# cvg/diffmvs

Hardware: AMD Instinct MI355X
Metric: depth-maps/sec (640x512, 5 src views) (higher is better)
Workload: dtype f32

## Files before the change

diffmvs_amd/_lib.py:

```python
from __future__ import annotations

import ctypes as C
import os

PKG = os.path.dirname(os.path.abspath(__file__))
HIP_LIB_PATH = os.environ.get("DMVS_LIB") or os.path.join(PKG, "libdmvs_hip.so")

ACT_NONE, ACT_RELU, ACT_SIGMOID, ACT_TANH, ACT_SILU = range(5)
IN_PLAIN, IN_UPSAMPLE2, IN_UNSHUFFLE2, IN_ZEROINSERT2 = range(4)
LAYOUT_NCHW, LAYOUT_NHWC, LAYOUT_NHWC_BF16, LAYOUT_NHWC_F16 = 0, 1, 2, 3
DTYPE_F32, DTYPE_BF16, DTYPE_F16, DTYPE_F32_PLAIN = 0, 1, 2, 3
ARITH_F32, ARITH_BF16, ARITH_SPLIT = 0, 1, 2
EW_DEPTH_TO_DISP, EW_DISP_TO_DEPTH = 0, 1

_P = C.c_void_p
_I = C.c_int32
_F = C.c_float


class Conv2dDesc(C.Structure):
    _fields_ = [
        ("in0", _P), ("in1", _P), ("mul0", _P), ("weight", _P), ("scale", _P), ("shift", _P),
        ("residual", _P), ("gru_z", _P), ("gru_h", _P), ("out", _P), ("gn_stats", _P), ("out_mul", _P),
        ("B", _I), ("c0", _I), ("c1", _I), ("Hin", _I), ("Win", _I), ("Hout", _I), ("Wout", _I),
        ("cout", _I), ("cout_pad", _I), ("kh", _I), ("kw", _I), ("stride", _I), ("pad_h", _I), ("pad_w", _I),
        ("in_mode", _I), ("act", _I), ("res_mode", _I), ("res_after_act", _I),
        ("out_layout", _I), ("out_cstride", _I), ("out_coffset", _I), ("gn_groups", _I), ("post_scale", _F),
        ("gate_cstride", _I), ("arith", _I), ("tune", _I), ("out_mul_c0", _I), ("in0_cstride", _I), ("weight_split", _P),
    ]


class Conv3dDesc(C.Structure):
    _fields_ = [
        ("in_", _P), ("weight", _P), ("scale", _P), ("shift", _P), ("residual", _P), ("out", _P),
        ("B", _I), ("cin", _I), ("cout", _I), ("cout_pad", _I),
        ("Din", _I), ("Hin", _I), ("Win", _I), ("Dout", _I), ("Hout", _I), ("Wout", _I),
        ("stride", _I), ("transposed", _I), ("act", _I), ("tune", _I),
    ]


class GetCostDesc(C.Structure):
    _fields_ = [
        ("ref", _P), ("src", _P), ("rt", _P), ("inv_depth", _P), ("confidence", _P), ("view_w", _P),
        ("disp_min", _P), ("disp_max", _P), ("out_cost", _P), ("out_samples", _P), ("worklist", _P),
        ("B", _I), ("S", _I), ("C", _I), ("G", _I), ("n", _I), ("H", _I), ("W", _I), ("vw_shift", _I),
        ("cost_cstride", _I), ("cost_coffset", _I), ("samp_cstride", _I), ("samp_coffset", _I),
        ("interval", _F), ("min_radius", _F), ("max_radius", _F), ("feat_dtype", _I), ("tune", _I),
    ]


SIGNATURES = {
    "dmvs_abi_version": [],
    "dmvs_conv2d_f32": [C.POINTER(Conv2dDesc), _P],
    "dmvs_featurenet_stem_f32": [_P, _P, _P, _P, _P, _P, _P, _P, _I, _I, _I, _I, _P],
    "dmvs_featurenet_stem3_f32": [_P, _P, _P, _P, _P, _P, _P, _P, _P, _P, _P, _I, _I, _I, _I, _P],
    "dmvs_conv2d_wgrad_workspace_f32": [C.POINTER(Conv2dDesc), C.POINTER(C.c_int64)],
    "dmvs_conv2d_wgrad_f32": [C.POINTER(Conv2dDesc), _P, _P, _P, _P, C.c_int64, _P],
    "dmvs_conv3d_f32": [C.POINTER(Conv3dDesc), _P],
    "dmvs_conv3d_wgrad_workspace_f32": [C.POINTER(Conv3dDesc), C.POINTER(C.c_int64)],
    "dmvs_conv3d_wgrad_f32": [C.POINTER(Conv3dDesc), _P, _P, _P, _P, C.c_int64, _P],
    "dmvs_compose_proj_f32": [_P, _P, _I, _I, _P],
    "dmvs_warp_volume_f32": [_P, _P, _P, _P, _I, _I, _I, _I, _I, _I, _I, _P],
    "dmvs_getcost_quad_f32": [C.POINTER(GetCostDesc), _P],
    "dmvs_warp_corr_init_quad_f32": [_P, _P, _P, _P, _P, _P, _I, _I, _I, _I, _I, _I, _I, _I, _I, _I, _I, _P],
    "dmvs_warp_corr_init_bwd_f32": [_P, _P, _P, _P, _P, _P, _P, _P, _I, _I, _I, _I, _I, _I, _I, _I, _I, _I, _P],
    "dmvs_getcost_bwd_f32": [C.POINTER(GetCostDesc), _P, _P, _P, _P],
    "dmvs_view_aggregate_bwd_f32": [_P, _P, _P, _P, _P, _P, _I, _I, _I, _I, _P],
    "dmvs_view_aggregate_f32": [_P, _P, _P, _I, _I, _I, _I, _P],
    "dmvs_sigmoid_max_d_f32": [_P, _P, _I, _I, _I, _P],
    "dmvs_depth_regress_f32": [_P, _P, _P, _P, _P, _P, _I, _I, _I, _P],
    "dmvs_convex_upsample_f32": [_P, _P, _P, _P, _P, _P, _I, _I, _I, _I, _P],
    "dmvs_mask_upsample4_f32": [_P, _P, _P, _F, _P, _P, _P, _P, _P, _I, _I, _I, _I, _I, _P],
    "dmvs_groupnorm_silu_f32": [_P, _P, _P, _P, _P, _P, _P, _I, _I, _I, _I, _F, _P],
    "dmvs_groupnorm_apply_f32": [_P, _P, _P, _P, _P, _P, _P, _I, _I, _I, _I, _F, _P],
    "dmvs_delta_update_f32": [_P, _P, _P, _F, _P, _P, _P, _I, _I, _I, _I, _P],
    "dmvs_depth_convert_f32": [_P, _P, _P, _P, _I, _I, _I, _P],
    "dmvs_act_slice_f32": [_P, _P, _I, _I, _I, _I, _I, _I, _I, _I, _P],
    "dmvs_upsample_nearest_f32": [_P, _P, _I, _I, _I, _I, _P],
    "dmvs_nchw_to_nhwc_f32": [_P, _P, _I, _I, _I, _P],
    "dmvs_groupnorm_silu_bwd_workspace_f32": [_I, _I, _I, C.POINTER(C.c_int64)],
    "dmvs_groupnorm_silu_bwd_f32": [_P, _P, _P, _P, _P, _P, _P, _P, _P, _P, _P, C.c_int64, _I, _I, _I, _I, _F, _P],
    "dmvs_batchnorm_workspace_f32": [_I, _I, _I, _I, C.POINTER(C.c_int64)],
    "dmvs_batchnorm_train_fwd_f32": [_P, _P, _P, _P, _P, _P, _P, _P, _P, C.c_int64, _I, _I, _I, _I, _I, _F, _F, _I, _P],
    "dmvs_batchnorm_train_bwd_f32": [_P, _P, _P, _P, _P, _P, _P, _P, _P, _P, C.c_int64, _I, _I, _I, _I, _I, _I, _P],
    "dmvs_geo_consistency_f32": [_P, _P, _P, _P, _P, _I, _I, _F, _F, _P, _P, _I, _I, _I, _I, _I, _P],
    "dmvs_sumsq_f32": [_P, C.c_int64, _P, _P],
    "dmvs_adamw_step_f32": [_P, _P, _P, _P, C.c_int64, _F, _F, _F, _F, _F, _I, _F, _P, _F, _P],
    "dmvs_view_select_scores_f64": [_P, _P, _P, _P, _P, C.c_int64, C.c_int64, _P, _I, C.c_double, C.c_double, C.c_double, _P, _P, _P],
    "dmvs_cloud_nn_dist_f32": [_P, C.c_int64, _P, C.c_int64, _P, _P, C.c_int64, _P, C.c_double, _P, _F, _P, _P, _P],
    "dmvs_cloud_stats_f32": [_P, _P, C.c_int64, _F, _P, _I, C.c_double, _I, _P, _P],
    "dmvs_cloud_nn_index_f32": [_P, C.c_int64, _P, C.c_int64, _P, _P, C.c_int64, _P, C.c_double, _P, _F, _P, _P, _P, _P, _P],
    "dmvs_cloud_pair_moments_f64": [_P, C.c_int64, _P, _P, C.c_int64, _P, _P, _F, _P, _P, C.c_double, C.c_double, C.c_double, _I, _P, _P],
    "dmvs_cloud_crop_prism_f32": [_P, C.c_int64, _P, _P, _I, _I, C.c_double, C.c_double, _P, _P],
    "dmvs_depth_stats_f32": [_P, _P, _P, C.c_int64, C.c_int64, _P, _I, C.c_double, C.c_double, C.c_double, C.c_double, _I, _P, _P],
    "dmvs_cloud_splat_zmin_f32": [_P, C.c_int64, _P, _P, C.c_int64, _I, _I, C.c_double, C.c_double, C.c_double, _I, _I, _P, _P, _P, _P],
    "dmvs_cloud_splat_sum_f32": [_P, C.c_int64, _P, _P, C.c_int64, _I, _I, C.c_double, C.c_double, C.c_double, C.c_double, C.c_double, _I, _P, _P, _P, _P],
    "dmvs_depth_normals_f32": [_P, _P, _P, C.c_int64, _I, _I, _I, C.c_double, _I, _P, _P, _P],
}
VIEW_SELECT_MAX_IMAGES, VIEW_SELECT_MAX_LIST = 16384, 1 << 23
CLOUD_MAX_RINGS, CLOUD_MAX_KEY_BITS, CLOUD_MAX_THRESHOLDS = 1024, 62, 16
CLOUD_MOMENTS, CLOUD_MAX_POLYGON = 20, 256
DEPTH_MAX_THRESHOLDS, DEPTH_SLOTS = 8, 7
SPLAT_VIEW_CHUNK, SPLAT_VIEW_DOUBLES, SPLAT_SLOTS, SPLAT_MAX_RADIUS, SPLAT_NO_PRETEST = 8, 15, 4, 16, 0x1
NORMAL_MAX_RADIUS, NORMAL_CAM_DOUBLES, NORMAL_VIEW_CHUNK, NORMAL_SLOTS = 4, 27, 8, 4
ABI_VERSION = 4
TUNE_NO_WALK, TUNE_PIECES4, TUNE_NO_LEAN, TUNE_1X1_TILED, TUNE_NO_TALL, TUNE_TALL = 0x4, 0x8, 0x100, 0x200, 0x400, 0x800
TUNE3D_PIECES4, TUNE3D_S2_DIRECT, TUNE3D_NO_PAIR = 0x1, 0x2, 0x4
TUNE_SWEEP_GLOBAL = 0x1
TUNE_WGRAD_ACCUMULATE = 0x1000
TUNE_SPLIT_ALL = 0x20000
TUNE_STEM_EXACT = 0x40000


def tune_xcd_group(n: int) -> int:
    return (int(n) & 7) << 14


def tune3d_xcd_group(n: int) -> int:
    return (int(n) & 7) << 4
TUNE_BWD_INTERLEAVED, BWD_GATHER_INTERLEAVED = 0x1, 2


def tune_tile_wx(n: int) -> int:
    return n & 3


def tune_tile_mt(n: int) -> int:
    return (n & 7) << 4


class DmvsError(RuntimeError):
    pass


class Lib:

    def __init__(self, path: str):
        if not os.path.exists(path):
# ... 27 lines not shown
```

diffmvs_amd/build.py:

```python
from __future__ import annotations

import os
import subprocess
import sys

PKG = os.path.dirname(os.path.abspath(__file__))
ROOT = os.path.dirname(PKG)
CSRC = os.path.join(PKG, "csrc")
LIB = os.path.join(PKG, "libdmvs_hip.so")
PROBE_LIB = os.path.join(PKG, "libdmvs_probe.so")
PROBE_SOURCES = ["probe/getcost_probe.hip", "probe/random_line_gather.hip"]
SOURCES = ["conv2d_k33.hip", "conv2d_k55.hip", "conv2d_k77.hip", "conv2d_k15.hip", "conv2d.hip", "stem.hip", "stem3.hip", "conv3d.hip", "warp_quad.hip", "warp_bwd.hip", "warp_bwd_win.hip", "warp_init_bwd_win.hip", "misc.hip", "mask_upsample.hip", "optim.hip", "norm.hip", "fusion.hip", "view_select.hip", "cloud_eval.hip", "cloud_register.hip", "depth_eval.hip", "cloud_render.hip", "depth_normals.hip"]


def _deps():
    out = [os.path.join(ROOT, "include", "dmvs.h"), os.path.join(ROOT, "include", "dmvs_probe.h")]
    for base, _, files in os.walk(CSRC):
        out += [os.path.join(base, f) for f in files]
    return out


def _stale() -> bool:
    if not os.path.exists(LIB) or not os.path.exists(PROBE_LIB):
        return True
    t = min(os.path.getmtime(LIB), os.path.getmtime(PROBE_LIB))
    return any(os.path.getmtime(d) > t for d in _deps())


def build_hip(force: bool = False, save_temps: bool = False, verbose: bool = True) -> str:
    if not force and not _stale():
        return LIB
    import time
    t_start = time.time()
    hipcc = os.environ.get("HIPCC", "/opt/rocm/bin/hipcc")
    flags = ["--offload-arch=gfx950", "-O3", "-std=c++17", "-fPIC",
             "-I", os.path.join(ROOT, "include"), "-I", CSRC,
             "-munsafe-fp-atomics",
             "-Wall", "-Wno-unused-function"]
    objdir = os.path.join(ROOT, "build", "temps" if save_temps else "obj")
    os.makedirs(objdir, exist_ok=True)
    if save_temps:
        flags += ["-save-temps=obj", "-Rpass-analysis=kernel-resource-usage"]

    hdr_t = max(os.path.getmtime(d) for d in _deps() if d.endswith(".h"))

    def compile_one(src):
        obj = os.path.join(objdir, src.replace("/", "_") + ".o")
        if not force and not save_temps and os.path.exists(obj) and os.path.getmtime(obj) > max(hdr_t, os.path.getmtime(os.path.join(CSRC, src))):
            return obj
        cmd = [hipcc] + flags + ["-c", os.path.join(CSRC, src), "-o", obj]
        if verbose:
            print("[diffmvs_amd.build]", " ".join(cmd), flush=True)
        t0 = time.time()
        subprocess.run(cmd, check=True, cwd=objdir if save_temps else ROOT)
        os.utime(obj, (t0, t0))
        return obj

    from concurrent.futures import ThreadPoolExecutor
    with ThreadPoolExecutor(max_workers=min(len(SOURCES), os.cpu_count() or 4)) as pool:
        objs = list(pool.map(compile_one, SOURCES + PROBE_SOURCES))
    for lib, lobjs in ((LIB, objs[:len(SOURCES)]), (PROBE_LIB, objs[len(SOURCES):])):
        link = [hipcc, "--offload-arch=gfx950", "-shared", "-fPIC"] + lobjs + ["-o", lib]
        if verbose:
            print("[diffmvs_amd.build]", " ".join(link), flush=True)
        subprocess.run(link, check=True, cwd=ROOT)
        os.utime(lib, (t_start, t_start))
    return LIB


if __name__ == "__main__":
    build_hip(force="--force" in sys.argv, save_temps="--save-temps" in sys.argv)
    print(LIB)
```

diffmvs_amd/engine.py:

```python
from __future__ import annotations

import math
import os
from typing import Callable, Dict, List, Optional

import torch
import torch.nn.functional as F

from . import ops as K
from .ops import Ops, PackedConv, pack_conv2d, pack_conv3d

_RATIOS = [4, 2, 1]
_MULTS = [(1,), (1, 2), (1, 2, 4)]


def _bn(sd, p):
    return {k: sd[f"{p}.{k}"] for k in ("weight", "bias", "running_mean", "running_var")}


def _cw(sd, p, **kw):
    return pack_conv2d(sd[p + ".conv.weight"], sd.get(p + ".conv.bias"),
                       bn=_bn(sd, p + ".bn") if (p + ".bn.weight") in sd else None, **kw)


def pack_feature(sd, p="feature", g4=False, feat_dtype=torch.float32):
    order = (lambda w: w[K.g4_channels(w.shape[0], feat_dtype).to(w.device)].contiguous()) if g4 else (lambda w: w)
    f = {"conv0.0": _cw(sd, p + ".conv0.0", pad=1), "conv0.1": _cw(sd, p + ".conv0.1", pad=1)}
    for i in (1, 2, 3):
        f[f"conv{i}.0"] = _cw(sd, f"{p}.conv{i}.0", stride=2, pad=2)
        f[f"conv{i}.1"], f[f"conv{i}.2"] = _cw(sd, f"{p}.conv{i}.1", pad=1), _cw(sd, f"{p}.conv{i}.2", pad=1)
    f["out1"] = pack_conv2d(order(sd[p + ".out1.weight"]))
    f["inner1"] = pack_conv2d(sd[p + ".inner1.weight"], sd[p + ".inner1.bias"])
    f["out2"] = pack_conv2d(order(sd[p + ".out2.weight"]), pad=1)
    if (p + ".out3.weight") in sd:
        f["inner2"] = pack_conv2d(sd[p + ".inner2.weight"], sd[p + ".inner2.bias"])
        f["out3"] = pack_conv2d(order(sd[p + ".out3.weight"]), pad=1)
    return f


STEM_FUSE_DEFAULT = "1"


def stem3_applies(o: Ops, x):
    return (o.conv_arith == K.ARITH_SPLIT and os.environ.get("DMVS_STEM_FUSE", STEM_FUSE_DEFAULT) != "0" and
            o.featurenet_stem3_supported(x))


def run_feature(o: Ops, f, x, layout=K.LAYOUT_NHWC, feat_dtype=torch.float32):
    R = K.ACT_RELU
    if stem3_applies(o, x):
        c1 = o.featurenet_stem3(f["conv0.0"], f["conv0.1"], f["conv1.0"], x)
    else:
        c0 = o.featurenet_stem(f["conv0.0"], f["conv0.1"], x)
        c1 = o.conv2d(f["conv1.0"], c0, act=R)
    c1 = o.conv2d(f["conv1.2"], o.conv2d(f["conv1.1"], c1, act=R), act=R)
    c2 = o.conv2d(f["conv2.2"], o.conv2d(f["conv2.1"], o.conv2d(f["conv2.0"], c1, act=R), act=R), act=R)
    c3 = o.conv2d(f["conv3.2"], o.conv2d(f["conv3.1"], o.conv2d(f["conv3.0"], c2, act=R), act=R), act=R)
    out = {"stage1": o.conv2d(f["out1"], c3, out_layout=layout, out_dtype=feat_dtype)}
    intra = o.conv2d(f["inner1"], c2, residual=c3, res_mode=K.IN_UPSAMPLE2)
    out["stage2"] = o.conv2d(f["out2"], intra, out_layout=layout, out_dtype=feat_dtype)
    if "out3" in f:
        intra = o.conv2d(f["inner2"], c1, residual=intra, res_mode=K.IN_UPSAMPLE2)
        out["stage3"] = o.conv2d(f["out3"], intra, out_layout=layout, out_dtype=feat_dtype)
    return out


def pack_context_trunk(sd, p="context"):
    c = {"conv1": _cw(sd, p + ".conv1", pad=1)}
    for li in (1, 2, 3):
        for bi in (0, 1):
            q = f"{p}.layer{li}.{bi}"
            c[f"{li}.{bi}.conv1"] = _cw(sd, q + ".conv1", stride=(2 if bi == 0 else 1), pad=1)
            c[f"{li}.{bi}.conv2"] = _cw(sd, q + ".conv2", pad=1)
            if bi == 0:
                c[f"{li}.{bi}.down"] = _cw(sd, q + ".downsample", stride=2, pad=1)
    return c


def run_context_trunk(o: Ops, c, x):
    R = K.ACT_RELU
    x = o.conv2d(c["conv1"], x, act=R)
    taps = {}
    for li in (1, 2, 3):
        y = o.conv2d(c[f"{li}.0.conv1"], x, act=R)
        xd = o.conv2d(c[f"{li}.0.down"], x)
        x = o.conv2d(c[f"{li}.0.conv2"], y, residual=xd, act=R)
        y = o.conv2d(c[f"{li}.1.conv1"], x, act=R)
        x = o.conv2d(c[f"{li}.1.conv2"], y, residual=x, act=R)
        taps[3 - li] = x
    return taps


def pack_pvw(sd, p):
    return (pack_conv3d(sd[p + ".conv.0.conv.weight"], bn=_bn(sd, p + ".conv.0.bn")),
            pack_conv3d(sd[p + ".conv.1.weight"], sd[p + ".conv.1.bias"]))


def run_pvw(o: Ops, pk, cor):
    N, _, D, H, W = cor.shape
    x = o.conv3d(pk[1], o.conv3d(pk[0], cor, act=K.ACT_RELU))
    return o.sigmoid_max_d(x.view(N, D, H, W))


def pack_costreg(sd, p):
    reg = {}
    for i, st in ((0, 1), (1, 1), (2, 2), (3, 1), (4, 2), (5, 1)):
        reg[i] = pack_conv3d(sd[f"{p}.conv{i}.conv.weight"], bn=_bn(sd, f"{p}.conv{i}.bn"), stride=st)
    for i in (6, 7):
        reg[i] = pack_conv3d(sd[f"{p}.conv{i}.conv.weight"], bn=_bn(sd, f"{p}.conv{i}.bn"), stride=2, transposed=True)
    reg["prob"] = pack_conv3d(sd[p + ".prob.weight"])
    return reg


def run_costreg(o: Ops, reg, x):
    R = K.ACT_RELU
    c1 = o.conv3d(reg[1], o.conv3d(reg[0], x, act=R), act=R)
    c3 = o.conv3d(reg[3], o.conv3d(reg[2], c1, act=R), act=R)
    x = o.conv3d(reg[5], o.conv3d(reg[4], c3, act=R), act=R)
    x = o.conv3d(reg[6], x, act=R, residual=c3)
    x = o.conv3d(reg[7], x, act=R, residual=c1)
    return o.conv3d(reg["prob"], x)


def pack_mask(sd, p):
    return (pack_conv2d(sd[p + ".0.weight"], sd[p + ".0.bias"], pad=1), pack_conv2d(sd[p + ".2.weight"], sd[p + ".2.bias"]))


def run_mask(o: Ops, pk, context, post_scale=0.25):
    return o.conv2d(pk[1], o.conv2d(pk[0], context, act=K.ACT_RELU), post_scale=post_scale)


def mask_head_fuses(pk, up_ratio) -> bool:
    return up_ratio == 4 and pk[1].cin == 64 and pk[1].cout == 144 and pk[1].scale is None and os.environ.get("DMVS_MASK_FUSE", "1") != "0"


def pack_gru(sd, p):
    g = {}
    for n, pad in (("1", (0, 2)), ("2", (2, 0))):
# ... 439 lines not shown
```

diffmvs_amd/ops.py:

```python
from __future__ import annotations

import ctypes as C
import os
from dataclasses import dataclass
from typing import Optional

import torch

from . import _lib
from ._lib import (ACT_NONE, ACT_RELU, ACT_SIGMOID, ACT_SILU, ACT_TANH, ARITH_BF16, ARITH_F32, ARITH_SPLIT, DTYPE_BF16, DTYPE_F16, DTYPE_F32, IN_PLAIN,
                   IN_UNSHUFFLE2, IN_UPSAMPLE2, IN_ZEROINSERT2, LAYOUT_NCHW, LAYOUT_NHWC, LAYOUT_NHWC_BF16, LAYOUT_NHWC_F16)

CONV_ARITH = {"fp32": ARITH_F32, "bf16": ARITH_BF16, "split": ARITH_SPLIT}
FEATURE_DTYPES = {"fp32": torch.float32, "bf16": torch.bfloat16, "fp16": torch.float16}
_DTYPE_CODE = {torch.float32: DTYPE_F32, torch.bfloat16: DTYPE_BF16, torch.float16: DTYPE_F16}
_NHWC_LAYOUT = {torch.float32: LAYOUT_NHWC, torch.bfloat16: LAYOUT_NHWC_BF16, torch.float16: LAYOUT_NHWC_F16}


def _round_up(x: int, m: int) -> int:
    return (x + m - 1) // m * m


@dataclass
class PackedConv:
# ... 246 lines not shown
            c0, Hin, Win = x0.shape[1], x0.shape[2] * 2, x0.shape[3] * 2
        else:
            c0, Hin, Win = x0.shape[1] * 4, x0.shape[2] // 2, x0.shape[3] // 2
        c1 = 0 if x1 is None else x1.shape[1]
        assert c0 + c1 == pc.cin, (c0, c1, pc.cin)
        kh, kw = pc.k
        Hout = (Hin + 2 * pc.pad[0] - kh) // pc.stride + 1
        Wout = (Win + 2 * pc.pad[1] - kw) // pc.stride + 1
        if out_cstride is None:
            out_cstride = pc.cout
        if out is None:
            shape = (B, out_cstride, Hout, Wout) if out_layout == LAYOUT_NCHW else (B, Hout, Wout, out_cstride)
            out = self.empty(*shape, dtype=out_dtype)
        arith = self.conv_arith if arith is None else arith
        wsplit = split_weights(pc) if (arith == ARITH_SPLIT and kh * kw > 1 and out_layout in (LAYOUT_NCHW, LAYOUT_NHWC)) else None
        d = _lib.Conv2dDesc(
            weight_split=_ptr(wsplit),
            in0=_ptr(x0), in1=_ptr(x1), mul0=_ptr(mul0), weight=_ptr(pc.weight), scale=_ptr(pc.scale),
            shift=_ptr(pc.shift), residual=_ptr(residual), gru_z=_ptr(gru_z), gru_h=_ptr(gru_h), out=_ptr(out),
            gn_stats=_ptr(gn_stats), gn_groups=(gn_groups if gn_stats is not None else 0), B=B, c0=c0, c1=c1, Hin=Hin, Win=Win, Hout=Hout, Wout=Wout, cout=pc.cout, cout_pad=pc.cout_pad,
            kh=kh, kw=kw, stride=pc.stride, pad_h=pc.pad[0], pad_w=pc.pad[1], in_mode=in_mode, act=act,
            res_mode=res_mode, res_after_act=int(res_after_act), out_layout=out_layout, out_cstride=out_cstride,
            out_coffset=out_coffset, post_scale=post_scale, gate_cstride=gate_cstride,
            arith=arith, tune=(self.tune["conv2d"] if tune is None else tune),
            out_mul=_ptr(out_mul), out_mul_c0=out_mul_c0, in0_cstride=in0_cstride)
        self._call("dmvs_conv2d_f32", C.byref(d), self.stream())
        if self.timers is not None and "dmvs_conv2d_f32" in self.timers:
            self.timers.setdefault("_conv2d_flops", []).append(2.0 * B * Hout * Wout * pc.cout * pc.cin * kh * kw)
            self.timers.setdefault("_conv2d_shape", []).append((B, pc.cin, pc.cout, kh, kw, pc.stride, Hout, Wout, in_mode, int(mul0 is not None)))
            nb = sum(t.numel() * t.element_size() for t in (x0, x1, mul0, residual, gru_z, gru_h, out_mul) if t is not None)
            self.timers.setdefault("_conv2d_bytes", []).append(nb + B * Hout * Wout * pc.cout * out.element_size())
        return out

    def featurenet_stem(self, pc0: PackedConv, pc1: PackedConv, x, tune=None):
        if isinstance(x, (list, tuple)):
            self._chk(*x)
            Bv, cin, H, W = x[0].shape
            y = self.empty(len(x) * Bv, 8, H, W)
            for v, xv in enumerate(x):
                self._stem_launch(pc0, pc1, xv, y[v * Bv:(v + 1) * Bv], tune)
            return y
        self._chk(x)
        N, cin, H, W = x.shape
        y = self.empty(N, 8, H, W)
        self._stem_launch(pc0, pc1, x, y, tune)
        return y

    def _stem_launch(self, pc0: PackedConv, pc1: PackedConv, x, y, tune=None):
        N, cin, H, W = x.shape
        if not (cin == 3 and pc0.cin == 3 and pc0.cout == 8 and pc1.cin == 8 and pc1.cout == 8 and pc0.k == (3, 3) and
                pc1.k == (3, 3) and pc0.stride == 1 and pc1.stride == 1 and pc0.pad == (1, 1) and pc1.pad == (1, 1) and
                pc0.cout_pad == 8 and pc1.cout_pad == 8):
            raise _lib.DmvsError("featurenet_stem: expects the 3->8->8 3x3 stem of FeatureNet")
        tune = self.tune["stem"] if tune is None else tune
        if self.conv_arith != ARITH_SPLIT:
            tune |= _lib.TUNE_STEM_EXACT
        self._call("dmvs_featurenet_stem_f32", _ptr(x), _ptr(pc0.weight), _ptr(pc0.scale), _ptr(pc0.shift), _ptr(pc1.weight),
                   _ptr(pc1.scale), _ptr(pc1.shift), _ptr(y), N, H, W, tune, self.stream())

    @staticmethod
    def featurenet_stem3_supported(x):
        xs = x if isinstance(x, (list, tuple)) else [x]
        H, W = xs[0].shape[2], xs[0].shape[3]
        return H % 2 == 0 and W % 4 == 0 and 3 * H * W < 2 ** 31 and all(t.data_ptr() % 16 == 0 for t in xs)

    def featurenet_stem3(self, pc0: PackedConv, pc1: PackedConv, pc2: PackedConv, x, tune=None):
        xs = x if isinstance(x, (list, tuple)) else [x]
        self._chk(*xs)
        Bv, cin, H, W = xs[0].shape
        if not (cin == 3 and pc0.cin == 3 and pc0.cout == 8 and pc1.cin == 8 and pc1.cout == 8 and pc0.k == (3, 3) and
                pc1.k == (3, 3) and pc0.stride == 1 and pc1.stride == 1 and pc0.pad == (1, 1) and pc1.pad == (1, 1) and
                pc0.cout_pad == 8 and pc1.cout_pad == 8 and pc2.cin == 8 and pc2.cout == 16 and pc2.cout_pad == 16 and pc2.k == (5, 5) and
                pc2.stride == 2 and pc2.pad == (2, 2)):
            raise _lib.DmvsError("featurenet_stem3: expects the 3->8->8 3x3 stem of FeatureNet and its 8->16 5x5 stride-2 conv1.0")
        if not self.featurenet_stem3_supported(xs) or any(t.shape != xs[0].shape for t in xs):
            raise _lib.DmvsError(f"featurenet_stem3: needs even H, W % 4 == 0 and 16-byte aligned views of one shape, got {tuple(xs[0].shape)}")
        y = self.empty(len(xs) * Bv, 16, H // 2, W // 2)
        for v, xv in enumerate(xs):
            self._call("dmvs_featurenet_stem3_f32", _ptr(xv), _ptr(pc0.weight), _ptr(pc0.scale), _ptr(pc0.shift), _ptr(pc1.weight),
                       _ptr(pc1.scale), _ptr(pc1.shift), _ptr(pc2.weight), _ptr(pc2.scale), _ptr(pc2.shift), _ptr(y[v * Bv:(v + 1) * Bv]),
                       Bv, H, W, 0 if tune is None else tune, self.stream())
        return y

    def conv2d_wgrad(self, pc: PackedConv, x0, grad_out, x1=None, *, mul0=None, in_mode=IN_PLAIN, want_bias=False, tune=None,
                     into_gw=None, into_gb=None):
        self._chk(x0, x1, mul0, grad_out, into_gw, into_gb)
        B = x0.shape[0]
        if in_mode == IN_PLAIN:
            c0, Hin, Win = x0.shape[1], x0.shape[2], x0.shape[3]
        elif in_mode in (IN_UPSAMPLE2, IN_ZEROINSERT2):
            c0, Hin, Win = x0.shape[1], x0.shape[2] * 2, x0.shape[3] * 2
        else:
            c0, Hin, Win = x0.shape[1] * 4, x0.shape[2] // 2, x0.shape[3] // 2
        c1 = 0 if x1 is None else x1.shape[1]
        kh, kw = pc.k
        Hout, Wout = grad_out.shape[2], grad_out.shape[3]
        acc = into_gw is not None
        if acc and (tuple(into_gw.shape) != (pc.cout, pc.cin, kh, kw) or (want_bias and (into_gb is None or tuple(into_gb.shape) != (pc.cout,)))):
            raise _lib.DmvsError("conv2d_wgrad: into_gw / into_gb do not have the gradient's shape")
        gw = into_gw if acc else self.empty(pc.cout, pc.cin, kh, kw)
        gb = (into_gb if acc else self.empty(pc.cout)) if want_bias else None
        d = _lib.Conv2dDesc(
            in0=_ptr(x0), in1=_ptr(x1), mul0=_ptr(mul0), weight=None, scale=None, shift=None, residual=None, gru_z=None,
            gru_h=None, out=None, gn_stats=None, gn_groups=0, B=B, c0=c0, c1=c1, Hin=Hin, Win=Win, Hout=Hout, Wout=Wout,
            cout=pc.cout, cout_pad=pc.cout_pad, kh=kh, kw=kw, stride=pc.stride, pad_h=pc.pad[0], pad_w=pc.pad[1],
            in_mode=in_mode, act=ACT_NONE, res_mode=IN_PLAIN, res_after_act=0, out_layout=LAYOUT_NCHW,
            out_cstride=pc.cout, out_coffset=0, post_scale=1.0, gate_cstride=0, arith=ARITH_F32,
            tune=((self.tune["conv2d"] & _lib.TUNE_PIECES4) if tune is None else tune) | (_lib.TUNE_WGRAD_ACCUMULATE if acc else 0))
        nbytes = C.c_int64(0)
        self._call("dmvs_conv2d_wgrad_workspace_f32", C.byref(d), C.byref(nbytes))
        ws = self.empty(nbytes.value // 4)
        self._call("dmvs_conv2d_wgrad_f32", C.byref(d), _ptr(grad_out), _ptr(gw), _ptr(gb), _ptr(ws), nbytes.value, self.stream())
        if self.timers is not None and "dmvs_conv2d_wgrad_f32" in self.timers:
            self.timers.setdefault("_wgrad_flops", []).append(2.0 * B * Hout * Wout * pc.cout * pc.cin * kh * kw)
        return (gw, gb) if want_bias else gw

    def conv3d(self, pc: PackedConv, x, *, act=ACT_NONE, residual=None, out=None, tune=None):
        self._chk(x, residual, out)
        B, cin, Din, Hin, Win = x.shape
        assert cin == pc.cin
        if pc.transposed:
            Dout, Hout, Wout = 2 * Din, 2 * Hin, 2 * Win
        else:
            s = pc.stride
            Dout, Hout, Wout = (Din - 1) // s + 1, (Hin - 1) // s + 1, (Win - 1) // s + 1
        if out is None:
            out = self.empty(B, pc.cout, Dout, Hout, Wout)
        d = _lib.Conv3dDesc(in_=_ptr(x), weight=_ptr(pc.weight), scale=_ptr(pc.scale), shift=_ptr(pc.shift),
                            residual=_ptr(residual), out=_ptr(out), B=B, cin=cin, cout=pc.cout, cout_pad=pc.cout_pad,
                            Din=Din, Hin=Hin, Win=Win, Dout=Dout, Hout=Hout, Wout=Wout, stride=pc.stride,
                            transposed=int(pc.transposed), act=act, tune=(self.tune["conv3d"] if tune is None else tune))
        self._call("dmvs_conv3d_f32", C.byref(d), self.stream())
        return out

    def conv3d_wgrad(self, x, grad_out, cout, stride, want_bias=False):
        self._chk(x, grad_out)
        B, cin, Din, Hin, Win = x.shape
        Dout, Hout, Wout = grad_out.shape[2:]
        gw = self.empty(cout, cin, 3, 3, 3)
        gb = self.empty(cout) if want_bias else None
        d = _lib.Conv3dDesc(in_=_ptr(x), weight=None, scale=None, shift=None, residual=None, out=None, B=B, cin=cin,
                            cout=cout, cout_pad=_pad_cout(cout), Din=Din, Hin=Hin, Win=Win, Dout=Dout, Hout=Hout, Wout=Wout,
                            stride=stride, transposed=0, act=ACT_NONE)
        nbytes = C.c_int64(0)
        self._call("dmvs_conv3d_wgrad_workspace_f32", C.byref(d), C.byref(nbytes))
        ws = self.empty(nbytes.value // 4)
        self._call("dmvs_conv3d_wgrad_f32", C.byref(d), _ptr(grad_out), _ptr(gw), _ptr(gb), _ptr(ws), nbytes.value, self.stream())
        return (gw, gb) if want_bias else gw

    def compose_proj(self, proj):
        self._chk(proj)
        B, V = proj.shape[0], proj.shape[1]
        out = self.empty(B, V - 1, 12)
        self._call("dmvs_compose_proj_f32", _ptr(proj), _ptr(out), B, V, self.stream())
        return out

    def warp_corr_init_quad(self, ref, src, rt, disp_min, disp_max, D, G=4, tune=None, plain=False):
        self._chk(rt, disp_min, disp_max)
        fdt = self._chk_feat(ref, src)
        if plain and fdt == DTYPE_F32:
            fdt = _lib.DTYPE_F32_PLAIN
        B, H, W, Cc = ref.shape
        S, _, Hs, Ws, _ = src.shape
        out = self.empty(B, S, G, D, H, W)
        self._call("dmvs_warp_corr_init_quad_f32", _ptr(ref), _ptr(src), _ptr(rt), _ptr(disp_min), _ptr(disp_max), _ptr(out),
                   B, S, Cc, G, D, H, W, Hs, Ws, fdt, self.tune["sweep"] if tune is None else tune, self.stream())
# ... 441 lines not shown
```

include/dmvs.h:

```cpp
#ifndef DMVS_H
#define DMVS_H

#include <stdint.h>

#ifdef __cplusplus
extern "C" {
#endif

#define DMVS_ABI_VERSION 4
#define DMVS_EINVAL (-22)

enum { DMVS_ACT_NONE = 0, DMVS_ACT_RELU = 1, DMVS_ACT_SIGMOID = 2, DMVS_ACT_TANH = 3, DMVS_ACT_SILU = 4 };
enum { DMVS_IN_PLAIN = 0, DMVS_IN_UPSAMPLE2 = 1 , DMVS_IN_UNSHUFFLE2 = 2 ,
       DMVS_IN_ZEROINSERT2 = 3  };
enum { DMVS_LAYOUT_NCHW = 0, DMVS_LAYOUT_NHWC = 1,
       DMVS_LAYOUT_NHWC_BF16 = 2, DMVS_LAYOUT_NHWC_F16 = 3 };
enum { DMVS_DTYPE_F32 = 0 , DMVS_DTYPE_BF16 = 1, DMVS_DTYPE_F16 = 2 ,
       DMVS_DTYPE_F32_PLAIN = 3  };

int dmvs_abi_version(void);

#define DMVS_ARITH_F32 0
#define DMVS_ARITH_BF16 1
#define DMVS_ARITH_SPLIT 2

#define DMVS_TUNE_TILE_WX(n) ((n) & 3)
#define DMVS_TUNE_NO_WALK 0x4
#define DMVS_TUNE_PIECES4 0x8
#define DMVS_TUNE_TILE_MT(n) (((n) & 7) << 4)
#define DMVS_TUNE_1X1_TILED 0x200
#define DMVS_TUNE_NO_LEAN 0x100
#define DMVS_TUNE_TALL(n) (((n) & 3) << 10)
#define DMVS_TUNE_STEM_EXACT 0x40000
#define DMVS_TUNE_SPLIT_ALL 0x20000
#define DMVS_TUNE_XCD_GROUP(n) (((n) & 7) << 14)

typedef struct dmvs_conv2d_desc {
    const float* in0;
    const float* in1;
    const float* mul0;
    const float* weight;
    const float* scale;
    const float* shift;
    const float* residual;
    const float* gru_z;
    const float* gru_h;
    float* out;
    double* gn_stats;
    const float* out_mul;
    int32_t B, c0, c1;
    int32_t Hin, Win;
    int32_t Hout, Wout;
    int32_t cout, cout_pad;
    int32_t kh, kw, stride, pad_h, pad_w;
    int32_t in_mode, act;
    int32_t res_mode;
    int32_t res_after_act;
    int32_t out_layout, out_cstride, out_coffset;
    int32_t gn_groups;
    float post_scale;
    int32_t gate_cstride;
    int32_t arith;
    int32_t tune;
    int32_t out_mul_c0;
    int32_t in0_cstride;
    const void* weight_split;
} dmvs_conv2d_desc;

int dmvs_conv2d_f32(const dmvs_conv2d_desc* d, void* stream);

int dmvs_featurenet_stem_f32(const float* x, const float* w0, const float* scale0, const float* shift0, const float* w1,
                             const float* scale1, const float* shift1, float* y, int32_t N, int32_t H, int32_t W, int32_t tune,
                             void* stream);

int dmvs_featurenet_stem3_f32(const float* x, const float* w0, const float* scale0, const float* shift0, const float* w1,
                              const float* scale1, const float* shift1, const float* w2, const float* scale2, const float* shift2,
                              float* y, int32_t N, int32_t H, int32_t W, int32_t tune, void* stream);

#define DMVS_TUNE_WGRAD_ACCUMULATE 0x1000
int dmvs_conv2d_wgrad_workspace_f32(const dmvs_conv2d_desc* d, int64_t* bytes);
int dmvs_conv2d_wgrad_f32(const dmvs_conv2d_desc* d, const float* grad_out, float* gw, float* gb, float* workspace,
                          int64_t workspace_bytes, void* stream);

typedef struct dmvs_conv3d_desc {
    const float* in;
    const float* weight;
    const float* scale;
    const float* shift;
    const float* residual;
    float* out;
    int32_t B, cin, cout, cout_pad;
    int32_t Din, Hin, Win;
    int32_t Dout, Hout, Wout;
    int32_t stride;
    int32_t transposed;
    int32_t act;
    int32_t tune;
} dmvs_conv3d_desc;
#define DMVS_TUNE3D_PIECES4 0x1
#define DMVS_TUNE3D_S2_DIRECT 0x2
#define DMVS_TUNE3D_NO_PAIR 0x4
#define DMVS_TUNE3D_XCD_GROUP(n) (((n) & 7) << 4)

int dmvs_conv3d_f32(const dmvs_conv3d_desc* d, void* stream);

int dmvs_conv3d_wgrad_workspace_f32(const dmvs_conv3d_desc* d, int64_t* bytes);
int dmvs_conv3d_wgrad_f32(const dmvs_conv3d_desc* d, const float* grad_out, float* gw, float* gb, float* workspace,
                          int64_t workspace_bytes, void* stream);

int dmvs_compose_proj_f32(const float* proj, float* out, int32_t B, int32_t V, void* stream);

#define DMVS_GETCOST_TILE 16
#define DMVS_GETCOST_MAX_WINDOW_VIEWS 16
#define DMVS_GETCOST_WORKLIST_INTS(B, H, W) \
    (4 + 66 * (B) * (((H) + DMVS_GETCOST_TILE - 1) / DMVS_GETCOST_TILE) * (((W) + DMVS_GETCOST_TILE - 1) / DMVS_GETCOST_TILE))
typedef struct dmvs_getcost_desc {
    const float* ref;
    const float* src;
    const float* rt;
    const float* inv_depth;
    const float* confidence;
    const float* view_w;
    const float* disp_min;
    const float* disp_max;
    float* out_cost;
    float* out_samples;
    int32_t* worklist;
    int32_t B, S, C, G, n, H, W;
    int32_t vw_shift;
    int32_t cost_cstride, cost_coffset, samp_cstride, samp_coffset;
    float interval, min_radius, max_radius;
    int32_t feat_dtype;
    int32_t tune;
} dmvs_getcost_desc;

#define DMVS_TUNE_SWEEP_GLOBAL 0x1
int dmvs_getcost_quad_f32(const dmvs_getcost_desc* d, void* stream);
int dmvs_warp_corr_init_quad_f32(const void* ref, const void* src, const float* rt,
                                 const float* disp_min, const float* disp_max, float* out,
                                 int32_t B, int32_t S, int32_t C, int32_t G, int32_t D,
                                 int32_t H, int32_t W, int32_t Hs, int32_t Ws, int32_t feat_dtype, int32_t tune, void* stream);

int dmvs_warp_volume_f32(const float* src, const float* rt, const float* depth, float* out,
                         int32_t B, int32_t C, int32_t D, int32_t H, int32_t W, int32_t Hs, int32_t Ws,
                         void* stream);

#define DMVS_TUNE_BWD_INTERLEAVED 0x1
#define DMVS_BWD_GATHER_INTERLEAVED 2
int dmvs_warp_corr_init_bwd_f32(const float* ref, const float* src, const float* rt,
                                const float* disp_min, const float* disp_max, const float* gcor,
                                float* gref, float* gsrc, int32_t B, int32_t S, int32_t C, int32_t G,
                                int32_t D, int32_t H, int32_t W, int32_t Hs, int32_t Ws, int32_t gather, void* stream);
int dmvs_getcost_bwd_f32(const dmvs_getcost_desc* d, const float* gcost, float* gref, float* gsrc, void* stream);
int dmvs_view_aggregate_bwd_f32(const float* cor, const float* w, const float* out, const float* gout,
                                float* gcor, float* gw, int32_t B, int32_t S, int32_t GD, int32_t HW,
                                void* stream);

int dmvs_view_aggregate_f32(const float* cor, const float* w, float* out,
                            int32_t B, int32_t S, int32_t GD, int32_t HW, void* stream);

int dmvs_sigmoid_max_d_f32(const float* x, float* out, int32_t N, int32_t D, int32_t HW, void* stream);
// ... 121 lines not shown
```

Baseline: 1484.

## Fuse FeatureNet conv1.1 and conv1.2 into one persistent producer-consumer kernel

Adds a persistent HIP kernel that runs the two 16->16 3x3 conv layers of FeatureNet conv1 back to back in a single launch. Half the waves compute layer one into an LDS ring of bf16-split rows, and the other half consume that ring for layer two, while async global-to-LDS loads stage the input. This removes the intermediate activation's round trip through global memory and one kernel launch, at the cost of a complex wave-specialised schedule with fixed strip sizes. It is enabled by default when split arithmetic is in use.

New measurement: 1518 (median of 6 runs). 1.02x the previous value.

```diff
diff --git a/diffmvs_amd/_lib.py b/diffmvs_amd/_lib.py
--- a/diffmvs_amd/_lib.py
+++ b/diffmvs_amd/_lib.py
@@ -54,6 +54,7 @@
     "dmvs_conv2d_f32": [C.POINTER(Conv2dDesc), _P],
     "dmvs_featurenet_stem_f32": [_P, _P, _P, _P, _P, _P, _P, _P, _I, _I, _I, _I, _P],
     "dmvs_featurenet_stem3_f32": [_P, _P, _P, _P, _P, _P, _P, _P, _P, _P, _P, _I, _I, _I, _I, _P],
+    "dmvs_featurenet_conv1_pair_f32": [_P, _P, _P, _P, _P, _P, _P, _P, _I, _I, _I, _I, _P],
     "dmvs_conv2d_wgrad_workspace_f32": [C.POINTER(Conv2dDesc), C.POINTER(C.c_int64)],
     "dmvs_conv2d_wgrad_f32": [C.POINTER(Conv2dDesc), _P, _P, _P, _P, C.c_int64, _P],
     "dmvs_conv3d_f32": [C.POINTER(Conv3dDesc), _P],
diff --git a/diffmvs_amd/build.py b/diffmvs_amd/build.py
--- a/diffmvs_amd/build.py
+++ b/diffmvs_amd/build.py
@@ -10,7 +10,7 @@
 LIB = os.path.join(PKG, "libdmvs_hip.so")
 PROBE_LIB = os.path.join(PKG, "libdmvs_probe.so")
 PROBE_SOURCES = ["probe/getcost_probe.hip", "probe/random_line_gather.hip"]
-SOURCES = ["conv2d_k33.hip", "conv2d_k55.hip", "conv2d_k77.hip", "conv2d_k15.hip", "conv2d.hip", "stem.hip", "stem3.hip", "conv3d.hip", "warp_quad.hip", "warp_bwd.hip", "warp_bwd_win.hip", "warp_init_bwd_win.hip", "misc.hip", "mask_upsample.hip", "optim.hip", "norm.hip", "fusion.hip", "view_select.hip", "cloud_eval.hip", "cloud_register.hip", "depth_eval.hip", "cloud_render.hip", "depth_normals.hip"]
+SOURCES = ["conv2d_k33.hip", "conv2d_k55.hip", "conv2d_k77.hip", "conv2d_k15.hip", "conv2d.hip", "stem.hip", "stem3.hip", "conv1_pair.hip", "conv3d.hip", "warp_quad.hip", "warp_bwd.hip", "warp_bwd_win.hip", "warp_init_bwd_win.hip", "misc.hip", "mask_upsample.hip", "optim.hip", "norm.hip", "fusion.hip", "view_select.hip", "cloud_eval.hip", "cloud_register.hip", "depth_eval.hip", "cloud_render.hip", "depth_normals.hip"]
 
 
 def _deps():
diff --git a/diffmvs_amd/csrc/conv1_pair.hip b/diffmvs_amd/csrc/conv1_pair.hip
--- /dev/null
+++ b/diffmvs_amd/csrc/conv1_pair.hip
@@ -0,0 +1,267 @@
+
+#include "dmvs_common.h"
+#include "dmvs_bf16.h"
+#include "dmvs_lds_poison.h"
+
+namespace {
+
+typedef float f32x4 __attribute__((ext_vector_type(4)));
+typedef uint32_t u32x4s __attribute__((ext_vector_type(4)));
+
+constexpr int PB = 512;
+constexpr int US = 80, UR = 64;
+constexpr int NP = US + 4;
+constexpr int SLOTS = 4;
+constexpr int PLQ = SLOTS * 2 * NP;
+constexpr int RINGQ = 3 * PLQ;
+constexpr int NLOAD = 2 * 2 * NP;
+constexpr int SW = US + 8;
+constexpr int STAGEF = 2 * 16 * SW;
+constexpr int NPIECE = STAGEF / 4;
+
+__device__ __attribute__((aligned(16))) const float conv1_pair_zero16[4] = {0.0f, 0.0f, 0.0f, 0.0f};
+#define DMVS_LDS_P(p) ((__attribute__((address_space(3))) void*)(p))
+#ifdef DMVS_HOST_EMULATION
+#define DMVS_OPAQUE(v) ((void)0)
+#else
+#define DMVS_OPAQUE(v) asm volatile("" : "+v"(v))
+#endif
+
+__global__ void __launch_bounds__(PB) __attribute__((amdgpu_waves_per_eu(4, 4)))
+featurenet_conv1_pair_kernel(const float* __restrict__ x, const u32x4s* __restrict__ ws1, const float* __restrict__ scale1,
+                             const float* __restrict__ shift1, const u32x4s* __restrict__ ws2, const float* __restrict__ scale2,
+                             const float* __restrict__ shift2, float* __restrict__ y, int N, int H, int W, int nsx, int nsy) {
+    __shared__ __attribute__((aligned(16))) float lds[2 * RINGQ * 4 + STAGEF];
+    DMVS_LDS_POISON(lds);
+
+    const int tid = threadIdx.x, lane = tid & 63, wave = __builtin_amdgcn_readfirstlane(tid >> 6);
+    const int m = lane & 15, kq = lane >> 4;
+    const int role = wave >> 2, wr = wave & 3;
+    const long plane = (long)H * W;
+    const int iplane = H * W;
+    const int nunits = nsx * nsy * N;
+
+    const u32x4s* const wsp = role ? ws2 : ws1;
+    u32x4s wq[2][3][3];
+#pragma unroll
+    for (int c = 0; c < 2; ++c)
+#pragma unroll
+        for (int g = 0; g < 3; ++g)
+#pragma unroll
+            for (int pl = 0; pl < 3; ++pl) wq[c][g][pl] = wsp[(((c * 3 + g) * 3 + pl) * 4 + kq) * 16 + m];
+    const float* const scp = role ? scale2 : scale1;
+    const float* const shp = role ? shift2 : shift1;
+    const float sc = scp ? scp[m] : 1.0f, sh = shp ? shp[m] : 0.0f;
+    int taps = 0;
+#pragma unroll
+    for (int g = 0; g < 3; ++g) {
+        const int t = min(4 * g + kq, 8);
+        taps |= ((t / 3) | ((t % 3) << 2)) << (4 * g);
+    }
+    const u32x4s* const src = reinterpret_cast<const u32x4s*>(lds) + role * RINGQ;
+    u32x4s* const in_q = reinterpret_cast<u32x4s*>(lds);
+    uint16_t* const mid_h = reinterpret_cast<uint16_t*>(lds) + RINGQ * 8;
+    float* const stage = lds + 2 * RINGQ * 4;
+    const int pmax = role ? US - 1 : US + 1;
+
+    const int tb = tid - PB / 2;
+    int lm = m, ltb = tb;
+
+    for (int unit = blockIdx.x; unit < nunits; unit += gridDim.x) {
+        const int sx = unit % nsx;
+        const int uq = unit / nsx;
+        const int sy = uq % nsy, n = uq / nsy;
+        const int X0 = US * sx, Y0 = UR * sy;
+        const int Yend = min(Y0 + UR, H) - 1;
+        const int nsteps = ((Yend - Y0 + 2) >> 1) + 4;
+        const float* const xb = x + (long)n * 16 * plane;
+        float* const yb = y + (long)n * 16 * plane;
+        const int row_lo = role ? Y0 : max(Y0 - 1, 0), row_hi = role ? Yend : min(Yend + 1, H - 1);
+        const int wlim = min(US, W - X0) + (role ? 0 : 2);
+        auto conv_group = [&](int row, int cg) -> f32x4 {
+            const int p = min(cg * 16 + lm, pmax);
+            bf16x8 ph[2], pm, pl;
+            auto qp_of = [&](int s) {
+                const int c = s / 3, g = s - c * 3;
+                const int tg = taps >> (4 * g);
+                const int slot = (row + 3 + (tg & 3)) & 3;
+                return (slot * 2 + c) * NP + p + ((tg >> 2) & 3);
+            };
+            {
+                const int qp = qp_of(0);
+                pl = __builtin_bit_cast(bf16x8, src[2 * PLQ + qp]);
+                ph[0] = __builtin_bit_cast(bf16x8, src[qp]);
+                pm = __builtin_bit_cast(bf16x8, src[PLQ + qp]);
+            }
+            f32x4 a = {0.0f, 0.0f, 0.0f, 0.0f};
+#pragma unroll
+            for (int s = 0; s < 6; ++s) {
+                const int b = s & 1, c = s / 3, g = s - c * 3;
+                const int qn = s + 1 < 6 ? qp_of(s + 1) : 0;
+                const bf16x8 wh = __builtin_bit_cast(bf16x8, wq[c][g][0]), wm = __builtin_bit_cast(bf16x8, wq[c][g][1]),
+                             wl = __builtin_bit_cast(bf16x8, wq[c][g][2]);
+                __builtin_amdgcn_sched_barrier(0);
+                a = dmvs_mfma_bf16(pl, wh, a);
+                __builtin_amdgcn_sched_barrier(0);
+                if (s + 1 < 6) pl = __builtin_bit_cast(bf16x8, src[2 * PLQ + qn]);
+                __builtin_amdgcn_sched_barrier(0);
+                a = dmvs_mfma_bf16(ph[b], wl, a);
+                a = dmvs_mfma_bf16(pm, wm, a);
+                a = dmvs_mfma_bf16(pm, wh, a);
+                __builtin_amdgcn_sched_barrier(0);
+                if (s + 1 < 6) {
+                    ph[b ^ 1] = __builtin_bit_cast(bf16x8, src[qn]);
+                    pm = __builtin_bit_cast(bf16x8, src[PLQ + qn]);
+                }
+                __builtin_amdgcn_sched_barrier(0);
+                a = dmvs_mfma_bf16(ph[b], wm, a);
+                a = dmvs_mfma_bf16(ph[b], wh, a);
+                __builtin_amdgcn_sched_barrier(0);
+            }
+            return a;
+        };
+        if (role) {
+            for (int j = 0; j < nsteps; ++j) {
+                const int lrow0 = Y0 - 2 + 2 * j;
+                DMVS_OPAQUE(lm);
+                DMVS_OPAQUE(ltb);
+#pragma unroll
+                for (int k = 0; k < 3; ++k) {
+                    const int e = k * (PB / 2) + ltb;
+                    if (k * (PB / 2) + wr * 64 < NPIECE) {
+                        const int li = e / (NPIECE / 2), rem = e - li * (NPIECE / 2);
+                        const int ch = rem / (SW / 4), pc = rem - ch * (SW / 4);
+                        const int row = lrow0 + li, col = X0 - 4 + 4 * pc;
+                        const bool ok = row <= Yend + 2 && row >= 0 && row < H && col >= 0 && col < W;
+                        const float* srcp = ok ? xb + (ch * iplane + row * W + col) : conv1_pair_zero16;
+                        float* dstp = stage + (k * (PB / 2) + wr * 64) * 4;
+                        __builtin_amdgcn_global_load_lds(srcp, DMVS_LDS_P(dstp), 16, 0, 0);
+                    }
+                }
+                const int rowbase = Y0 + 2 * j - 8;
+                f32x4 acc[3];
+#pragma unroll
+                for (int i = 0; i < 3; ++i) {
+                    const int gi = wr + 4 * i;
+                    const int rr = gi >= 5 ? 1 : 0, cg = gi - rr * 5;
+                    const int row = rowbase + rr;
+                    acc[i] = f32x4{0.0f, 0.0f, 0.0f, 0.0f};
+                    if (gi < 10 && cg * 16 < wlim && row >= row_lo && row <= row_hi) acc[i] = conv_group(row, cg);
+                }
+                DMVS_DMA_BARRIER();
+#pragma unroll
+                for (int i = 0; i < 3; ++i) {
+                    const int gi = wr + 4 * i;
+                    const int rr = gi >= 5 ? 1 : 0, cg = gi - rr * 5;
+                    const int row = rowbase + rr;
+                    const int x0 = cg * 16 + 4 * kq, col = X0 + x0;
+                    if (gi < 10 && row >= row_lo && row <= row_hi && x0 < US && col < W) {
+                        f32x4 v;
+#pragma unroll
+                        for (int r = 0; r < 4; ++r) v[r] = fmaxf(acc[i][r] * sc + sh, 0.0f);
+                        *reinterpret_cast<f32x4*>(yb + (m * iplane + row * W + col)) = v;
+                    }
+                }
+                auto convert_item = [&](bool need, int li, int lc, int lq) {
+                    const int lrow = lrow0 + li;
+                    if (need && lrow <= Yend + 2) {
+                        const float* sp = stage + (li * 16 + lc * 8) * SW + lq + 2;
+                        float v[8];
+#pragma unroll
+                        for (int c8 = 0; c8 < 8; ++c8) v[c8] = sp[c8 * SW];
+                        bf16x8 h8, m8, l8;
+                        dmvs_split3_bf16x8(v, h8, m8, l8);
+                        u32x4s* const d = in_q + (((lrow + 4) & 3) * 2 + lc) * NP + lq;
+                        d[0] = __builtin_bit_cast(u32x4s, h8);
+                        d[PLQ] = __builtin_bit_cast(u32x4s, m8);
+                        d[2 * PLQ] = __builtin_bit_cast(u32x4s, l8);
+                    }
+                };
+                DMVS_OPAQUE(ltb);
+                const int li0 = ltb / (2 * NP), lrem = ltb - li0 * (2 * NP);
+                const int lc0 = lrem / NP;
+                convert_item(true, li0, lc0, lrem - lc0 * NP);
+                convert_item(ltb + PB / 2 < NLOAD, 1, 1, ltb + PB / 2 - 3 * NP);
+                DMVS_LDS_BARRIER();
+            }
+        } else {
+            for (int j = 0; j < nsteps; ++j) {
+                DMVS_OPAQUE(lm);
+                const int rowbase = Y0 + 2 * j - 5;
+                f32x4 acc[3];
+#pragma unroll
+                for (int i = 0; i < 3; ++i) {
+                    const int gi = wr * 3 + i;
+                    const int rr = gi >= 6 ? 1 : 0, cg = gi - rr * 6;
+                    const int row = rowbase + rr;
+                    acc[i] = f32x4{0.0f, 0.0f, 0.0f, 0.0f};
+                    if (cg * 16 < wlim && row >= row_lo && row <= row_hi) acc[i] = conv_group(row, cg);
+                }
+                DMVS_DMA_BARRIER();
+#pragma unroll
+                for (int i = 0; i < 3; ++i) {
+                    const int gi = wr * 3 + i;
+                    const int rr = gi >= 6 ? 1 : 0, cg = gi - rr * 6;
+                    const int row = rowbase + rr;
+                    if (row >= Y0 - 1 && row <= Yend + 1 && cg * 16 < wlim) {
+                        const int p0 = cg * 16 + 4 * kq;
+                        const bool rin = row >= 0 && row < H;
+                        float v[8];
+#pragma unroll
+                        for (int r = 0; r < 4; ++r) {
+                            const int col = X0 - 1 + p0 + r;
+                            const bool inside = rin && col >= 0 && col < W;
+                            v[r] = inside ? fmaxf(acc[i][r] * sc + sh, 0.0f) : 0.0f;
+                            v[4 + r] = 0.0f;
+                        }
+                        bf16x8 h8, m8, l8;
+                        dmvs_split3_bf16x8(v, h8, m8, l8);
+                        uint16_t* const d = mid_h + ((((row + 4) & 3) * 2 + (m >> 3)) * NP + p0) * 8 + (m & 7);
+#pragma unroll
+                        for (int r = 0; r < 4; ++r) {
+                            if (p0 + r < US + 2) {
+                                d[r * 8] = (uint16_t)h8[r];
+                                d[PLQ * 8 + r * 8] = (uint16_t)m8[r];
+                                d[2 * PLQ * 8 + r * 8] = (uint16_t)l8[r];
+                            }
+                        }
+                    }
+                }
+                DMVS_LDS_BARRIER();
+            }
+        }
+    }
+}
+
+#ifdef DMVS_HOST_EMULATION
+int conv1_pair_resident() { return 2; }
+#else
+int conv1_pair_resident() {
+    int dev = 0, per_cu = 0;
+    hipDeviceProp_t prop;
+    if (hipGetDevice(&dev) != hipSuccess || hipGetDeviceProperties(&prop, dev) != hipSuccess) return 512;
+    if (hipOccupancyMaxActiveBlocksPerMultiprocessor(&per_cu, reinterpret_cast<const void*>(featurenet_conv1_pair_kernel), PB, 0) != hipSuccess || per_cu < 1)
+        per_cu = 1;
+    return per_cu * prop.multiProcessorCount;
+}
+#endif
+
+}
+
+extern "C" int dmvs_featurenet_conv1_pair_f32(const float* x, const void* wsplit1, const float* scale1, const float* shift1, const void* wsplit2,
+                                              const float* scale2, const float* shift2, float* y, int32_t N, int32_t H, int32_t W, int32_t tune,
+                                              void* stream) {
+    if (!x || !wsplit1 || !wsplit2 || !y || N <= 0 || H <= 0 || W <= 0) return DMVS_EINVAL;
+    if ((long)16 * H * W >= (1L << 31)) return DMVS_EINVAL;
+    if ((W & 3) || (((uintptr_t)x | (uintptr_t)y | (uintptr_t)wsplit1 | (uintptr_t)wsplit2) & 15)) return DMVS_EINVAL;
+    const int nsx = (W + US - 1) / US, nsy = (H + UR - 1) / UR;
+    const long nunits = (long)nsx * nsy * N;
+    if (nunits >= (1L << 31)) return DMVS_EINVAL;
+    static const int resident = conv1_pair_resident();
+    long grid = (tune & 0xffff) ? (tune & 0xffff) : resident;
+    if (grid > nunits) grid = nunits;
+    hipLaunchKernelGGL(featurenet_conv1_pair_kernel, dim3((unsigned)grid), dim3(PB), 0, (hipStream_t)stream, x,
+                       reinterpret_cast<const u32x4s*>(wsplit1), scale1, shift1, reinterpret_cast<const u32x4s*>(wsplit2), scale2, shift2, y, N, H, W,
+                       nsx, nsy);
+    return dmvs_launch_status();
+}
diff --git a/diffmvs_amd/engine.py b/diffmvs_amd/engine.py
--- a/diffmvs_amd/engine.py
+++ b/diffmvs_amd/engine.py
@@ -46,6 +46,14 @@
             o.featurenet_stem3_supported(x))
 
 
+CONV1_PAIR_DEFAULT = "1"
+
+
+def conv1_pair_applies(o: Ops, c1):
+    return (o.conv_arith == K.ARITH_SPLIT and os.environ.get("DMVS_CONV1_PAIR", CONV1_PAIR_DEFAULT) != "0" and
+            o.conv1_pair_supported(c1) and c1.shape[3] >= K.Ops.CONV1_PAIR_STRIP)
+
+
 def run_feature(o: Ops, f, x, layout=K.LAYOUT_NHWC, feat_dtype=torch.float32):
     R = K.ACT_RELU
     if stem3_applies(o, x):
@@ -53,7 +61,10 @@
     else:
         c0 = o.featurenet_stem(f["conv0.0"], f["conv0.1"], x)
         c1 = o.conv2d(f["conv1.0"], c0, act=R)
-    c1 = o.conv2d(f["conv1.2"], o.conv2d(f["conv1.1"], c1, act=R), act=R)
+    if conv1_pair_applies(o, c1):
+        c1 = o.conv1_pair(f["conv1.1"], f["conv1.2"], c1)
+    else:
+        c1 = o.conv2d(f["conv1.2"], o.conv2d(f["conv1.1"], c1, act=R), act=R)
     c2 = o.conv2d(f["conv2.2"], o.conv2d(f["conv2.1"], o.conv2d(f["conv2.0"], c1, act=R), act=R), act=R)
     c3 = o.conv2d(f["conv3.2"], o.conv2d(f["conv3.1"], o.conv2d(f["conv3.0"], c2, act=R), act=R), act=R)
     out = {"stage1": o.conv2d(f["out1"], c3, out_layout=layout, out_dtype=feat_dtype)}
diff --git a/diffmvs_amd/ops.py b/diffmvs_amd/ops.py
--- a/diffmvs_amd/ops.py
+++ b/diffmvs_amd/ops.py
@@ -352,6 +352,26 @@
                        Bv, H, W, 0 if tune is None else tune, self.stream())
         return y
 
+    CONV1_PAIR_STRIP, CONV1_PAIR_SEGMENT = 80, 64
+
+    @staticmethod
+    def conv1_pair_supported(x):
+        return (x.dim() == 4 and x.shape[1] == 16 and x.shape[3] % 4 == 0 and 16 * x.shape[2] * x.shape[3] < 2 ** 31 and
+                x.data_ptr() % 16 == 0)
+
+    def conv1_pair(self, pc1: PackedConv, pc2: PackedConv, x, tune=0):
+        self._chk(x)
+        for pc in (pc1, pc2):
+            if not (pc.cin == 16 and pc.cout == 16 and pc.cout_pad == 16 and pc.k == (3, 3) and pc.stride == 1 and pc.pad == (1, 1)):
+                raise _lib.DmvsError("conv1_pair: expects the two 16->16 3x3 stride-1 layers of FeatureNet's conv1")
+        if not self.conv1_pair_supported(x):
+            raise _lib.DmvsError(f"conv1_pair: needs 16 channels, W % 4 == 0 and a 16-byte aligned tensor, got {tuple(x.shape)}")
+        N, _, H, W = x.shape
+        y = self.empty(N, 16, H, W)
+        self._call("dmvs_featurenet_conv1_pair_f32", _ptr(x), _ptr(split_weights(pc1)), _ptr(pc1.scale), _ptr(pc1.shift),
+                   _ptr(split_weights(pc2)), _ptr(pc2.scale), _ptr(pc2.shift), _ptr(y), N, H, W, tune, self.stream())
+        return y
+
     def conv2d_wgrad(self, pc: PackedConv, x0, grad_out, x1=None, *, mul0=None, in_mode=IN_PLAIN, want_bias=False, tune=None,
                      into_gw=None, into_gb=None):
         self._chk(x0, x1, mul0, grad_out, into_gw, into_gb)
diff --git a/include/dmvs.h b/include/dmvs.h
--- a/include/dmvs.h
+++ b/include/dmvs.h
@@ -77,6 +77,10 @@
                               const float* scale1, const float* shift1, const float* w2, const float* scale2, const float* shift2,
                               float* y, int32_t N, int32_t H, int32_t W, int32_t tune, void* stream);
 
+int dmvs_featurenet_conv1_pair_f32(const float* x, const void* wsplit1, const float* scale1, const float* shift1, const void* wsplit2,
+                                   const float* scale2, const float* shift2, float* y, int32_t N, int32_t H, int32_t W, int32_t tune,
+                                   void* stream);
+
 #define DMVS_TUNE_WGRAD_ACCUMULATE 0x1000
 int dmvs_conv2d_wgrad_workspace_f32(const dmvs_conv2d_desc* d, int64_t* bytes);
 int dmvs_conv2d_wgrad_f32(const dmvs_conv2d_desc* d, const float* grad_out, float* gw, float* gb, float* workspace,
```
